# NOAA-GFDL/GRTCODE

Hardware: AMD Instinct MI355X
Metric: columns/sec (60-layer, 1 cm⁻¹ LBL, LW+SW) (higher is better)
Workload: dtype f64

## Files before the change

### grtcode_amd/csrc/grt_kernels.h

```cpp
#ifndef GRT_KERNELS_H_
#define GRT_KERNELS_H_

#include <stddef.h>
#include <stdint.h>

#ifdef __cplusplus
extern "C" {
#endif

#define GRT_MAX_ISO 18
#define GRT_MAX_SLOTS 53
#define GRT_MAX_TABLES 32

typedef struct GrtLineStore
{
    uint64_t n;
    double const *v0;
    double const *s0;
    float const *yair;
    float const *yself;
    float const *en;
    float const *nexp;
    float const *delta;
    uint8_t const *iso;
// ... 33 lines not shown
    GrtLineStore lines;
    GrtColumnLayout lay;
    double const *colstate;
    double const *tables;
    double const *h2o_tables;
    double w0, wres;
    uint64_t nw;
    int ncol;
    double *tau;
    uint64_t tau_col_stride;
    int tile;
    int nslice;
    int fast;
    float *gmom;
    uint64_t gmom_stride;
    int halo;
    int rcap;
    int tree_levels;
    int mom_terms;
    int profile_tag;
    int near_block;
    int deterministic;
    unsigned long long *probe;
    int direct_near;
    int tile_phase, tile_nphase;
    uint32_t const *tile_ranges;
    int lean;
    uint32_t const *tile_items;
    uint32_t n_items;
    GrtTableSpans spans;
    int *radius_table;
    int skip_tables;
    int narrow;
} GrtGasOpticsArgs;

typedef struct GrtContinua
{
    double const *colstate;
    uint64_t stride, off_cont, off_h2o;
    double const *tables;
    double const *h2o_tables;
    int num_tables, has_h2o_ctm;
    GrtTableSpans spans;
} GrtContinua;
int grt_launch_add_continua(void *stream, GrtContinua const *c, int num_layers, int ncol, uint64_t nw,
                            double *tau_gas, uint64_t col_stride);


int grt_launch_gas_optics(void *stream, GrtGasOpticsArgs const *a);
enum { GRT_TAG_FAR_OFFSET = 5 };
int grt_profile_begin(void *stream, int tag);
void grt_profile_end(void *stream, int slot);
int grt_launch_gas_optics_mp(void *stream, GrtGasOpticsArgs const *a);
int grt_gas_optics_mp_shape(GrtGasOpticsArgs const *a);
int grt_gas_optics_lean_shape(GrtGasOpticsArgs const *a);
int grt_tree_gather_by_wave(long long fsteps);
uint64_t grt_gas_optics_moment_floats(uint64_t nw, int levels, int terms);
double grt_gas_optics_moment_separation(int terms);

typedef struct GrtSweepBins
{
    double w0, wres;
    uint64_t num_wpoints, n;
    int ppb, do_interp, do_last_interp;
    double const *w;
    double *tau;
    uint64_t const *l, *r;
} GrtSweepBins;
int grt_launch_sweep_sort(void *stream, uint64_t n, int num_layers, double const *v0, double shift_max,
                          double const *lay, double const *prep, double *sorted);
int grt_launch_sweep(void *stream, int method, uint64_t n, int num_layers, double const *lines,
                     double const *ns, GrtSweepBins const *bins, double *tau);
int grt_launch_sweep_interpolate(void *stream, int num_layers, GrtSweepBins const *bins, double *tau);

int grt_launch_line_prep(void *stream, GrtGasOpticsArgs const *a, int col,
                         double *vnn, double *snn, double *gamma, double *alpha,
                         int64_t *win_s, int64_t *win_e);

int grt_launch_voigt_debug(void *stream, int fast, double w_start, uint64_t n, double wres, double center,
                           double gamma, double alpha, double *K_dev);

int grt_launch_rayleigh(void *stream, int num_layers, double w0, double dw, uint64_t nw,
                        double const *n_layer_host, double *tau, double *omega, double *g);

typedef struct GrtOpticsPtrs { double const *tau[8]; double const *omega[8]; double const *g[8]; } GrtOpticsPtrs;
int grt_launch_add_optics(void *stream, uint64_t n, int num_optics, GrtOpticsPtrs const *in,
                          double *tau, double *omega, double *g);

// ... 293 lines not shown
```

### grtcode_amd/csrc/hip/gas_optics_mp_dev.h

```cpp
#ifndef GRT_GAS_OPTICS_MP_DEV_H_
#define GRT_GAS_OPTICS_MP_DEV_H_
#include <type_traits>
#include "gas_optics_dev.h"

namespace {

constexpr int kMom = 8;
constexpr int kFarGradedMin = 64;
constexpr int kMomWide = 12;

__host__ __device__ inline double moment_separation(int terms)
{
    return terms == kMomWide ? 3.95 : 7.8;
}
constexpr size_t kLdsPerWorkgroup = 64*1024;
constexpr int kRcap = 12;
constexpr int kPowTable = 128;
constexpr int kCellLoop = 3;

template <int CTRL>
__device__ __forceinline__ float dpp_f(float v)
{
    int const b = __float_as_int(v);
    return __int_as_float(__builtin_amdgcn_update_dpp(0, b, CTRL, 0xf, 0xf, true));
}

__device__ __forceinline__ double row_pass(double v)
{
    int lo = __double2loint(v), hi = __double2hiint(v);
    lo = __builtin_amdgcn_update_dpp(lo, lo, 0x121, 0xf, 0xf, false);
    hi = __builtin_amdgcn_update_dpp(hi, hi, 0x121, 0xf, 0xf, false);
    return __hiloint2double(hi, lo);
}

// ... 108 lines not shown
    for (int i = 0; i < 8; ++i)
    {
        w[i] = dpp_add_by_bit<8>(g0[i], g1[i]);
    }
    float x[4];
#pragma unroll
    for (int i = 0; i < 4; ++i)
    {
        x[i] = dpp_add_by_bit<4>(w[i], w[i + 4]);
    }
    float y[2];
#pragma unroll
    for (int i = 0; i < 2; ++i)
    {
        float const keep = b1 ? x[i + 2] : x[i];
        float const send = b1 ? x[i] : x[i + 2];
        y[i] = keep + dpp_f<0x1B>(send);
    }
    float const keep = b0 ? y[1] : y[0];
    float const send = b0 ? y[0] : y[1];
    return keep + dpp_f<0xB1>(send);
}

constexpr int kRawCap = 128;
constexpr int kLeanListCap = 12;
constexpr int kLeanMaxP = 4;
constexpr int kLeanSlots = 16;
struct LeanTables
{
    float ps[kLeanSlots], p_ps[kLeanSlots], dop[kLeanSlots];
    float qn_m[kLeanSlots*GRT_MAX_ISO], qn_e[kLeanSlots*GRT_MAX_ISO];
    float ptab[kPowTable];
};
struct LeanRaw
{
    unsigned long long xl_mask[kWaves][kLeanListCap][kLeanMaxP];
    unsigned j[kWaves][kRawCap];
    float amp[kWaves][kRawCap];
    float delta[kWaves][kRawCap];
    unsigned idx[kWaves][kRawCap];
    unsigned xl_base[kWaves][kLeanListCap];
};

constexpr int kClasses = 3;
constexpr int kClassesSplit = 4;
constexpr int kMpQueue = 64;
constexpr int kMpQueueTree = 64;

template <int CAP, int NCLS>
struct MpQueue
{
    static constexpr int capacity = CAP;
    static constexpr int classes = NCLS;
    float amp[NCLS][kWaves][CAP];
    float xi[NCLS][kWaves][CAP];
    float y[NCLS][kWaves][CAP];
    unsigned short idx[NCLS][kWaves][CAP];
};
using MpQueueFlat = MpQueue<kMpQueue, kClassesSplit>;
using MpQueueTree = MpQueue<kMpQueueTree, kClassesSplit>;

__device__ __attribute__((noinline)) double exp_fp64_call(double x)
{
    return exp_fp64(x);
}

// ... 152 lines not shown
```

### grtcode_amd/csrc/hip/k_gas_optics_far.hip

```cpp
#include "gas_optics_mp_dev.h"

namespace {

__global__ __launch_bounds__(kBlock) void near_radius_kernel(GrtGasOpticsArgs a, long long fsteps_ll, int cell_shift, int ntiles)
{
    extern __shared__ __attribute__((aligned(16))) unsigned char smem[];
    double *ms_l = reinterpret_cast<double *>(smem);
    double *q_l = ms_l + 4*a.lay.num_slots;
    int const tid = threadIdx.x;
    int const layer = blockIdx.x, col = blockIdx.y;
    double const *cs = a.colstate + (uint64_t)col*a.lay.stride;
    double const *lay = cs + a.lay.off_lay + (uint64_t)layer*4;
    stage_column_state(a, cs, layer, ms_l, q_l, tid);
    __syncthreads();
    long long const nw = (long long)a.nw;
    for (int t = tid; t < ntiles; t += kBlock)
    {
        long long const c1 = ((long long)(t + 1) << cell_shift);
        bool um, cr;
        int const R = near_radius(a, lay, ms_l, (long long)t << cell_shift, c1 < nw ? c1 : nw, (int)fsteps_ll, &um, &cr);
        long long const F1 = c1 < nw ? c1 : nw;
        unsigned const tf = lean_tile_flags(a, lay, ms_l, (int)((long long)t << cell_shift), (int)F1, cr);
        a.radius_table[((uint64_t)col*a.lay.num_layers + layer)*ntiles + t] = R | (um ? 0x10000 : 0) | (cr ? 0x20000 : 0) | (int)(tf << kTileFlagsShift);
    }
}

__global__ __launch_bounds__(kBlock) void gas_optics_far_kernel(GrtGasOpticsArgs a, long long fsteps_ll, int cell_shift, int ncell)
{
    extern __shared__ __attribute__((aligned(16))) unsigned char smem[];
    int const fsteps = (int)fsteps_ll;
    double *acc = reinterpret_cast<double *>(smem);
    double *ms_l = acc + a.tile;
    double *q_l = ms_l + 4*a.lay.num_slots;
    float *mom = reinterpret_cast<float *>(q_l + GRT_MAX_ISO*a.lay.num_slots);
    float *invr = mom + (size_t)kMom*ncell;
    int *rtab = reinterpret_cast<int *>(invr + fsteps + 1);
    int const tid = threadIdx.x;
    int const layer = blockIdx.y, col = blockIdx.z;
    long long const nw = (long long)a.nw;
    long long const F0l = (long long)blockIdx.x*a.tile;
    long long const F1l = (F0l + a.tile < nw) ? F0l + a.tile : nw;
    int const F0 = (int)F0l, F1 = (int)F1l;
    double const *cs = a.colstate + (uint64_t)col*a.lay.stride;
    double const *lay = cs + a.lay.off_lay + (uint64_t)layer*4;
    double *out = a.tau + (uint64_t)col*a.tau_col_stride + (uint64_t)layer*a.nw;
    bool const own_radii = a.radius_table == nullptr || fsteps > kFarGradedMin;
    if (own_radii)
// ... 703 lines not shown
    return sizeof(double)*tile + sizeof(double)*num_slots*(4 + GRT_MAX_ISO) + sizeof(float)*((size_t)kMom*ncell + fsteps + 1)
           + sizeof(int)*((size_t)(ncell >> cell_shift) + 3);
}

}

extern "C" size_t grt_far_lds_bytes(int tile, int ncell, int fsteps, int num_slots, int cell_shift)
{
    return far_lds_bytes(tile, ncell, fsteps, num_slots, cell_shift);
}

extern "C" size_t grt_tree_lds_bytes(int tile, int num_slots, int ntab)
{
    return tree_lds_bytes(tile, num_slots, ntab);
}

extern "C" int grt_tree_gather_tile(void)
{
    return tree_gather_tile();
}

extern "C" int grt_tree_gather_ntab(int tile, int halo)
{
    return tree_gather_ntab(tile, halo);
}

extern "C" int grt_tree_gather_by_wave(long long fsteps)
{
    return tree_gather_by_wave(fsteps) ? 1 : 0;
}

extern "C" int grt_launch_near_radius(void *stream, GrtGasOpticsArgs const *bp, long long fsteps, int shift)
{
    int const ntiles = (int)((bp->nw + ((uint64_t)1 << shift) - 1) >> shift);
    hipLaunchKernelGGL(near_radius_kernel, dim3(bp->lay.num_layers, bp->ncol), dim3(kBlock),
                       sizeof(double)*bp->lay.num_slots*(4 + GRT_MAX_ISO), (hipStream_t)stream, *bp, fsteps, shift, ntiles);
    return (int)hipGetLastError();
}

extern "C" int grt_launch_far_field(void *stream, GrtGasOpticsArgs const *bp, long long fsteps, int shift)
{
    hipStream_t const s = (hipStream_t)stream;
    GrtGasOpticsArgs b = *bp;
    if (b.tree_levels > 0)
    {
        int first_level = 1;
        while ((2 << (first_level - 1)) <= b.tile && first_level <= b.tree_levels) ++first_level;
        if (b.mom_terms == kMomWide)
        {
            launch_tree<kMomWide>(s, b, fsteps, shift, first_level);
        }
        else
        {
            launch_tree<kMom>(s, b, fsteps, shift, first_level);
        }
        return (int)hipGetLastError();
    }
    int const far_want = 512;
    int far_tile = b.tile;
    while (2*far_tile <= far_want && (uint64_t)far_tile < b.nw
           && far_lds_bytes(2*far_tile, 2*far_tile + 2*(int)fsteps, (int)fsteps, b.lay.num_slots, shift) <= kLdsPerWorkgroup)
    {
        far_tile *= 2;
    }
    b.tile = far_tile;
    unsigned const far_tiles = (unsigned)((b.nw + far_tile - 1)/far_tile);
    int const far_ncell = far_tile + 2*(int)fsteps;
    hipLaunchKernelGGL(gas_optics_far_kernel, dim3(far_tiles, b.lay.num_layers, b.ncol), dim3(kBlock),
                       far_lds_bytes(far_tile, far_ncell, (int)fsteps, b.lay.num_slots, shift), s, b, fsteps, shift, far_ncell);
    return (int)hipGetLastError();
// ... 2 lines not shown
```

### grtcode_amd/csrc/hip/k_gas_optics_mp.hip

```cpp
#include "gas_optics_mp_dev.h"

extern "C" size_t grt_far_lds_bytes(int tile, int ncell, int fsteps, int num_slots, int cell_shift);
extern "C" size_t grt_tree_lds_bytes(int tile, int num_slots, int ntab);
extern "C" int grt_tree_gather_tile(void);
extern "C" int grt_tree_gather_ntab(int tile, int halo);
extern "C" int grt_tree_gather_by_wave(long long fsteps);
extern "C" int grt_launch_far_field(void *stream, GrtGasOpticsArgs const *b, long long fsteps, int shift);
extern "C" int grt_launch_near_radius(void *stream, GrtGasOpticsArgs const *b, long long fsteps, int shift);

namespace {

template <int CLASS, int ONLY, bool PACKED4, typename Queue>
__device__ __forceinline__ void drain_class(double *acc, Queue const *q, int wave, int first, int count, int lane)
{
    for (int i = first + lane; i < first + count; i += 64)
    {
        float const xi = q->xi[CLASS][wave][i], y = q->y[CLASS][wave][i];
        unsigned const idx = q->idx[CLASS][wave][i];
        float const far = (idx & 0x8000u) ? (y*kRsqrpi)*__builtin_amdgcn_rcpf(fmaf(xi, xi, y*y)) : 0.f;
        double const k = voigt_near<true, ONLY, PACKED4>(xi, y) - (double)far;
        GRT_ACC_ADD(&acc[idx & 0x7fffu], (double)q->amp[CLASS][wave][i]*k);
    }
}

// ... 75 lines not shown
            if (tid == 0)
            {
                probe_rec[2] = nlines;
                probe_rec[3] = (unsigned long long)R | ((unsigned long long)corrected << 16) | ((unsigned long long)use_moments << 17);
                probe_rec[1] = __builtin_readcyclecounter();
            }
        }
    };
    int const cell0 = TWO_PASS ? F0 : F0 - fsteps;
    int const A0 = TWO_PASS ? F0 - halo : F0;

    double const *cs = a.colstate + (uint64_t)col*a.lay.stride;
    double const *lay = cs + a.lay.off_lay + (uint64_t)layer*4;

    for (int i = tid; i < nacc; i += kBlock)
    {
        acc[i] = 0.0;
    }
    for (int i = tid; i < kMom*ncell; i += kBlock)
    {
        mom[i] = 0.f;
    }
    if (TREE && K == kMomWide && ncell == 0)
    {
        for (int i = tid; i < 2*(a.tile >> 5); i += kBlock)
        {
            occ_any[i] = 0u;
        }
    }
    for (int i = tid; i <= fsteps && !TWO_PASS; i += kBlock)
    {
        invr[i] = i > 0 ? 1.0f/(float)i : 0.f;
    }
    stage_column_state(a, cs, layer, ms_l, q_l, tid);
    for (int i = tid; i < kPowTable; i += kBlock)
    {
        ptab[i] = exp_fp64((double)((float)i/100.f)*lay[3]);
    }
    if (TWO_PASS && a.tile_ranges != nullptr)
    {
        if (tid == 0 && a.tile_items != nullptr)
        {
            range[0] = (long long)a.tile_items[4*(uint64_t)wi.group + 1];
            range[1] = (long long)a.tile_items[4*(uint64_t)wi.group + 2];
        }
        else if (tid == 0)
        {
            uint64_t const jlo = a.tile_ranges[2*tile_idx], jhi = a.tile_ranges[2*tile_idx + 1];
            uint64_t const per = (jhi - jlo + a.nslice - 1)/a.nslice;
            uint64_t const b = jlo + per*slice;
            uint64_t e = b + per;
            if (e > jhi) e = jhi;
            range[0] = (long long)(b < jhi ? b : jhi);
            range[1] = (long long)e;
        }
    }
    else if (wave == 0)
    {
        candidate_range_wave(a, lay, F0l, F1l, TWO_PASS ? 0 : fsteps_ll, slice, range, lane);
    }
    __syncthreads();
    if constexpr (PROBE)
    {
        if (tid == 0) probe_rec[11] = __builtin_readcyclecounter();
    }
    uint64_t const jbeg = (uint64_t)range[0];
    uint64_t const jend = (uint64_t)range[1];

    float const wres_f = (float)a.wres;
    double const inv_wres = 1./a.wres;
// ... 510 lines not shown
    bool const tree = a->tree_levels > 0;
    if ((items && (a->fast != 3 || a->tile_ranges == nullptr || a->n_items == 0 || tree || a->deterministic || a->probe != NULL))
        || (a->lean && (a->probe != NULL || !grt_gas_optics_lean_shape(a))) || (a->narrow && (a->fast != 3 || tree))
        || (a->near_block != 0 && (a->near_block != 64 || !tree)))
    {
        return (int)hipErrorInvalidValue;
    }
    unsigned long long const ngroups = items ? a->n_items : tiles*a->nslice;
    unsigned long long const blocks = ngroups*a->lay.num_layers*a->ncol;
    if (blocks == 0 || blocks > 0x7fffffffull)
    {
        return (int)hipErrorInvalidValue;
    }
    hipStream_t const s = (hipStream_t)stream;
    if (a->fast == 3)
    {
        int const halo = a->halo;
        int const nacc = a->tile + 2*halo, shift = log2_exact(a->tile);
        if (a->ncol > 65535 || a->lay.num_layers > 65535 || (tree && a->nslice != 1))
        {
            return (int)hipErrorInvalidValue;
        }
        hipError_t e = hipMemsetAsync(a->tau, 0, sizeof(double)*a->tau_col_stride*(size_t)a->ncol, s);
        if (e == hipSuccess && a->nslice > 1)
        {
            e = hipMemsetAsync(a->gmom, 0, sizeof(float)*a->gmom_stride*a->lay.num_layers*a->ncol, s);
        }
        bool const wide = tree && a->mom_terms == kMomWide;
        if (e != hipSuccess)
        {
            return (int)e;
        }
        GrtGasOpticsArgs b = *a;
        if (!tree && b.radius_table != nullptr)
        {
            int const rc_radius = grt_launch_near_radius(stream, &b, fsteps, shift);
            if (rc_radius != 0)
            {
                return rc_radius;
            }
        }
        int slot = a->profile_tag ? grt_profile_begin(stream, a->profile_tag) : -1;
        int const ncell = (tree && a->tile > kDirectTile) ? 0 : a->tile;
        size_t lds = mp_lds_bytes(nacc, ncell, 0, a->lay.num_slots, tree, tree && ncell == 0 ? a->tile : 0);
        if (a->lean)
        {
            lds += lean_lds_bytes(a->lay.num_slots);
        }
        int const nphase = a->deterministic ? (2*halo)/a->tile + 2 : 1;
        if (a->deterministic && a->nslice != 1)
        {
            return (int)hipErrorInvalidValue;
        }
        void (*first_pass)(GrtGasOpticsArgs, long long, unsigned, unsigned, int, int, int);
        if (wide && a->probe != NULL) first_pass = gas_optics_mp_probe_wide_kernel;
        else if (wide) first_pass = gas_optics_mp_kernel<true, true, kMomWide>;
        else if (tree) first_pass = gas_optics_mp_kernel_w5<true, true, kMom>;
        else if (a->probe != NULL) first_pass = a->narrow ? gas_optics_mp_probe_kernel<true> : gas_optics_mp_probe_kernel<false>;
        else if (a->lean) first_pass = a->narrow ? gas_optics_lean_kernel<true> : gas_optics_lean_kernel<false>;
        else first_pass = a->narrow ? gas_optics_mp_kernel_w5<true, false, kMom, true> : gas_optics_mp_kernel_w5<true, false, kMom>;
        for (int phase = 0; phase < nphase; ++phase)
        {
            b.tile_phase = phase;
            b.tile_nphase = nphase;
            hipLaunchKernelGGL(first_pass, dim3((unsigned)blocks), dim3(kBlock), lds, s, b, fsteps, (unsigned)ngroups,
                               golden_stride(ngroups), ncell, nacc, halo);
        }
        if (a->profile_tag) grt_profile_end(stream, slot);
        b.nslice = 1;
        slot = a->profile_tag ? grt_profile_begin(stream, a->profile_tag + GRT_TAG_FAR_OFFSET) : -1;
        int const rc_far = grt_launch_far_field(stream, &b, fsteps, shift);
        if (a->profile_tag) grt_profile_end(stream, slot);
        return rc_far;
    }
    int const ncell = a->tile + 2*(int)fsteps;
// ... 6 lines not shown
```

### grtcode_amd/csrc/hip/mp_lean_block.inc

```

    static_assert(kLeanP == 2, "the lean loop keeps the two lines of a lane in the halves of packed registers");
    constexpr int kLinesPerLane = LEAN_LOOP ? kLeanP : 1;
    [[maybe_unused]] bool lean_ok = false;
    [[maybe_unused]] LeanTables *lt = nullptr;
    [[maybe_unused]] LeanRaw *raw = nullptr;
    [[maybe_unused]] int rawcount = 0;
    [[maybe_unused]] int xcount = 0;
    [[maybe_unused]] float kh = 0.f, kl = 0.f, c2t = 0.f, pw = 0.f, pavg_f = 0.f, a_norm = 0.f, wres_v = 0.f, inv_wres_v = 0.f;
    [[maybe_unused]] unsigned tflags = 0u;
    auto uniform_flag = [](bool b) { return __builtin_amdgcn_readfirstlane((int)b) != 0; };
    if constexpr (LEAN_LOOP)
    {
        size_t const lean_off = ((size_t)(reinterpret_cast<unsigned char *>(invr + 1) - smem) + 15) & ~(size_t)15;
        lt = reinterpret_cast<LeanTables *>(smem + lean_off);
        raw = reinterpret_cast<LeanRaw *>(lt + 1);
        lean_ok = uniform_flag(a.lean != 0 && use_moments && R == 3 && fsteps >= 8 && halo >= 8
                               && a.lines.lean_a != nullptr);
        if (lean_ok)
        {
            for (int i = tid; i < a.lay.num_slots; i += kBlock)
            {
                lt->ps[i] = (float)ms_l[4*i];
                lt->p_ps[i] = (float)ms_l[4*i + 1];
                lt->dop[i] = (float)(((double)0.83255461115f/(double)kSqrln2)*ms_l[4*i + 3]);
            }
            for (int i = tid; i < a.lay.num_slots*GRT_MAX_ISO; i += kBlock)
            {
                double const v = q_l[i]*ms_l[(i/GRT_MAX_ISO)*4 + 2];
                int e = 0;
                double const m = frexp(v, &e);
                bool const ok = v > 0. && v < 1e300;
                lt->qn_m[i] = ok ? (float)(2.*m) : 0.f;
                lt->qn_e[i] = ok ? (float)(e - 1 - GRT_LEAN_S0_SHIFT) : 0.f;
            }
            for (int i = tid; i < kPowTable; i += kBlock)
            {
                lt->ptab[i] = (float)ptab[i];
            }
            __syncthreads();
            double const kTd = ((double)(-1.4387686f)*1.4426950408889634)*lay[2];
            kh = (float)kTd;
            kl = (float)(kTd - (double)kh);
            c2t = (float)((double)(-1.4387686f)*lay[2]);
            pw = (float)(lay[0]*inv_wres);
            pavg_f = (float)lay[0];
            a_norm = (float)(1./(3.14159265358979323846*a.wres));
            wres_v = wres_f;
            inv_wres_v = inv_wres_f;
            asm volatile("" : "+v"(kh), "+v"(kl), "+v"(c2t), "+v"(pw), "+v"(pavg_f), "+v"(a_norm), "+v"(wres_v), "+v"(inv_wres_v));
            unsigned const tf = tile_flags_known ? tile_flags : lean_tile_flags(a, lay, ms_l, F0, F1, corrected);
            tflags = (unsigned)__builtin_amdgcn_readfirstlane((int)tf);
        }
    }

    uint64_t const jal = lean_ok ? (jbeg & ~(uint64_t)1) : jbeg;
    uint64_t const walk_first = a.deterministic ? (wave == 0 ? jal : jend) : jal + (uint64_t)wave*64*kLinesPerLane;
    unsigned const walk_stride = (a.deterministic ? 64u : (unsigned)kBlock)*kLinesPerLane;

    [[maybe_unused]] auto drain_raw = [&](int const first, int const count)
    {
        if constexpr (LEAN_LOOP)
        {
            bool const on = lane < count;
            int const i = first + (on ? lane : 0);
            unsigned const packed = raw->idx[wave][i];
            unsigned const j = raw->j[wave][i];
            int const idx = (int)(packed & 4095u);
            int const c = idx + A0 - ((int)((packed >> 12) & 15u) - 3);
            double2 const lx = reinterpret_cast<double2 const *>(a.lines.lean_x)[j];
            float const yair = __int_as_float(__double2loint(lx.y)), yself = __int_as_float(__double2hiint(lx.y));
            double const *ms = ms_l + ((packed >> 16) & 63u)*4;
            double const wnoadj = lx.x + (double)raw->delta[wave][i]*lay[0];
            int const s = c - fsteps < 0 ? 0 : c - fsteps;
            LineWidths const lw = reference_widths(ptab[(packed >> 22) & 127u], yair, yself, ms, wnoadj);
            float const repwid = lw.repwid, y = lw.y;
            double const dwno = (double)s*a.wres + a.w0;
            float const xr = voigt_x(dwno, idx + A0 - s, a.wres, wnoadj, repwid);
            int const cls = on ? voigt_class<true, kSplit>(xr, y) : -1;
            queue_push(cls, raw->amp[wave][i]*(kRsqrpi*repwid), xr, y, (unsigned short)idx);
        }
    };
// ... 439 lines not shown
```

### grtcode_amd/csrc/host/grt_gas_launch.c

```c
#include <math.h>
#include <stdlib.h>
#include <string.h>
#include "grt_internal.h"

#define TREE_MIN_FSTEPS 200
#define ITEM_LINES 10000u

typedef struct LaunchPlan
{
    GrtGasOpticsArgs a;
    int tables;
    int items;
    double pmax;
    size_t moment_bytes;
    size_t radius_bytes;
    uint64_t probe_words;
} LaunchPlan;

static void auto_tune(GasOptics_t const *go, int ncol, int moments, int *tile, int *nslice)
{
    GrtGasOpticsImpl const *im = impl_of(go);
    uint64_t const nw = go->grid.n;
    double const per_cell = nw > 0 ? (double)im->store.n/(double)nw : 0.;
    int t = im->tile;
    if (t == 0)
    {
        int want = moments == 2 ? 256 : (moments ? 512 : 1024);
        while (moments == 2 && want > (ncol == 1 ? 128 : 64) && per_cell*(double)(want/2) >= 6000.
               && ((nw + want - 1)/want)*(uint64_t)go->num_layers*(uint64_t)ncol < 16384)
        {
            want >>= 1;
        }
        t = nw >= (uint64_t)want ? want : (int)(((nw + 63)/64)*64);
        if (moments == 2)
        {
            while (t & (t - 1))
            {
                t += 64;
            }
        }
    }
    int ns = im->nslice;
    if (ns == 0)
    {
        uint64_t const blocks = ((nw + t - 1)/t)*(uint64_t)go->num_layers*(uint64_t)ncol;
        double const per_tile = per_cell*(double)t;
        ns = 1;
        while (blocks*ns < 16384 && ns < 16 && per_tile/(double)(2*ns) >= 8000.)
// ... 242 lines not shown
            }
            a->gmom_stride = grt_gas_optics_moment_floats(a->nw, a->tree_levels, a->mom_terms);
        }
        if (!grt_gas_optics_mp_shape(a))
        {
            a->fast = im->fast == 3 ? 1 : 2;
            a->tree_levels = 0;
            a->mom_terms = 0;
            a->rcap = 12;
            if (a->fast == 1)
            {
                auto_tune(go, ncol, 1, &a->tile, &a->nslice);
                if (!grt_gas_optics_mp_shape(a))
                {
                    a->fast = 2;
                }
            }
        }
    }
    if (a->fast != 1 && a->fast != 3)
    {
        auto_tune(go, ncol, 0, &a->tile, &a->nslice);
    }
    a->direct_near = a->fast == 1 || a->fast == 3;
    uint64_t const tiles = (a->nw + (uint64_t)a->tile - 1)/(uint64_t)a->tile;
    if (a->fast == 3)
    {
        char const *lean = getenv("GRT_LEAN");
        a->lean = !(lean != NULL && lean[0] == '0') && grt_gas_optics_lean_shape(a);
        a->narrow = a->tree_levels == 0 && a->w0 + (double)a->nw*a->wres <= 4000.;
        a->near_block = a->tree_levels > 0 && grt_tree_gather_by_wave(fsteps) ? 64 : 0;
        p->moment_bytes = sizeof(float)*(size_t)a->gmom_stride*(size_t)go->num_layers;
        p->radius_bytes = a->tree_levels == 0 ? sizeof(int)*(size_t)tiles*(size_t)go->num_layers : 0;
        if (a->tree_levels == 0 || a->mom_terms == 12)
        {
            p->probe_words = 24*tiles*(uint64_t)a->nslice*(uint64_t)go->num_layers;
        }
        p->tables = im->sorted_v0_h != NULL && im->store.n > 0 && im->store.n < 0xffffffffull;
        for (int c = 0; c < ncol && p->tables && im->colstate_h != NULL; ++c)
        {
            double const *lay = im->colstate_h + (size_t)c*im->layout.stride + im->layout.off_lay;
            for (int i = 0; i < go->num_layers; ++i)
            {
                p->pmax = fabs(lay[(size_t)i*4]) > p->pmax ? fabs(lay[(size_t)i*4]) : p->pmax;
            }
        }
        char const *env = getenv("GRT_TILE_ITEMS");
        p->items = p->tables && im->nslice == 0 && a->tree_levels == 0 && !grt_deterministic()
                   && !(env != NULL && env[0] == '0') && tiles*(uint64_t)go->num_layers*(uint64_t)ncol < 16384;
    }
    if (grt_deterministic())
    {
        a->deterministic = 1;
        a->nslice = 1;
    }
}

static int grow(GasOptics_t *go, void **buf, size_t *have, size_t need)
{
    if (need > *have)
    {
        GRT_TRY(grt_dev_free(go->device, *buf));
        *buf = NULL;
        *have = 0;
        GRT_TRY(grt_dev_alloc(go->device, buf, need));
        *have = need;
    }
    return GRTCODE_SUCCESS;
}

static int bind(GasOptics_t *go, LaunchPlan const *p, int c0, int ncol, double *tau, uint64_t tau_col_stride,
                GrtGasOpticsArgs *a)
{
    GrtGasOpticsImpl *im = impl_of(go);
    *a = p->a;
    a->ncol = ncol;
    a->colstate = im->colstate_d + (size_t)c0*im->layout.stride;
    a->tau = tau + (size_t)c0*tau_col_stride;
    a->tau_col_stride = tau_col_stride;
    if (p->moment_bytes > 0)
    {
        GRT_TRY(grow(go, (void **)&im->gmom, &im->gmom_bytes, p->moment_bytes*(size_t)ncol));
        a->gmom = im->gmom;
    }
    if (p->radius_bytes > 0)
    {
        GRT_TRY(grow(go, (void **)&im->radius_table, &im->radius_bytes, p->radius_bytes*(size_t)ncol));
        a->radius_table = im->radius_table;
    }
    if (im->probe != NULL && p->probe_words > 0 && p->probe_words*(uint64_t)ncol <= im->probe_words)
    {
        a->probe = im->probe;
        a->lean = 0;
    }
    if (p->tables)
    {
        GRT_TRY(tile_tables(go, a, p->pmax));
        a->tile_ranges = im->tile_ranges_d;
        if (p->items && a->probe == NULL && im->n_items > 0)
        {
            a->tile_items = im->tile_items_d;
            a->n_items = im->n_items;
            a->nslice = im->items_cut > 1 ? 2 : 1;
        }
    }
    return GRTCODE_SUCCESS;
}

static int launch_sweep_columns(GasOptics_t *go, int ncol, double *tau_dev, uint64_t tau_col_stride)
{
    GrtGasOpticsImpl *im = impl_of(go);
    void *s = grt_dev_stream(go->device);
    int const L = go->num_layers;
    uint64_t nmax = 0;
    for (int sl = 0; sl < go->num_molecules; ++sl)
    {
        if (im->mstore[sl].n > nmax) nmax = im->mstore[sl].n;
    }
    if (nmax > 0 && im->sweep_scratch == NULL)
    {
        GRT_TRY(grt_dev_alloc(go->device, (void **)&im->sweep_scratch, sizeof(double)*8*(size_t)L*nmax));
    }
    GRT_TRY(grt_gas_optics_upload_states(go, ncol));
    GrtSweepBins bins = {go->bins.w0, go->bins.wres, go->bins.num_wpoints, go->bins.n, go->bins.ppb,
                         go->bins.do_interp, go->bins.do_last_interp, go->bins.w, go->bins.tau, go->bins.l, go->bins.r};
    int const method = go->optical_depth_method == wavenumber_sweep ? 0 : 1;
// ... 125 lines not shown
```

### grtcode_amd/csrc/host/grt_gas_optics.c

```c
#include <math.h>
#include <stdio.h>
#include <stdlib.h>
#include <string.h>
#include "grt_internal.h"
#include "grt_molecule_table.h"

static double const MIN_CUTOFF = 1.;
static double const MAX_CUTOFF = 50.;
static double const DEFAULT_CUTOFF = 25.;

static char const *const cfc_names[NUM_CFCS] = {
    "CFC-11", "CFC-12", "CFC-113", "CFC-114", "CFC-115", "HCFC-22", "HCFC-141b", "HCFC-142b",
    "HFC-23", "HFC-125", "HFC-134a", "HFC-143a", "HFC-152a", "HFC-227ea", "HFC-245fa", "CCl4",
    "C2F6", "CF4", "CH2Cl2", "NF3", "SF6"};

int grt_load_table_on_grid(char const *path, int expect_cols, SpectralGrid_t const *grid, fp_t *out)
{
    int rows = 0, cols = 0;
    char **tok = NULL;
    GRT_TRY(parse_csv(path, &rows, &cols, 1, &tok));
    int rc = GRTCODE_SUCCESS;
    fp_t *vals = malloc(sizeof(fp_t)*(size_t)rows*(size_t)cols);
    for (int i = 0; i < rows*cols; ++i)
    {
// ... 162 lines not shown
        if (told != im->fast)
        {
            told = im->fast;
            GRT_INFO("Line kernel form %d (%s); GRT_GAS_OPTICS_FAST=0 or grt_gas_optics_tune selects the reference's operation order.",
                     im->fast, im->fast == 0 ? "reference operation order, tau within 1e-11"
                               : "fused arithmetic, tau within 2e-6 of each layer's maximum, sums in the scheduler's order");
        }
    }
    size_t const V = (size_t)num_levels;
    go->x = calloc(NUM_MOLS*V, sizeof(fp_t));
    go->x_cfc = calloc(NUM_CFCS*V, sizeof(fp_t));
    go->x_cia = calloc(NUM_CIAS*V, sizeof(fp_t));
    GRT_TRY(grt_dev_alloc(go->device, (void **)&im->lin_tables, sizeof(double)*GRT_MAX_TABLES*grid->n));
    im->store_dirty = 1;
    GRT_TRY(inittips_d());
    GRT_INFO("Gas optics on device %d: %d levels, %zu grid points.", go->device, num_levels, (size_t)grid->n);
    return GRTCODE_SUCCESS;
}

EXTERN int destroy_gas_optics(GasOptics_t * const gas_optics)
{
    GRT_REQUIRE_PTR(gas_optics);
    GrtGasOpticsImpl *im = impl_of(gas_optics);
    if (im != NULL)
    {
        for (int i = 0; i < NUM_MOLS; ++i)
        {
            grt_free_host_lines(&im->host[i]);
        }
        GRT_TRY(grt_free_line_store(gas_optics));
        GRT_TRY(grt_dev_free(gas_optics->device, im->bins_block));
        GRT_TRY(grt_dev_free(gas_optics->device, im->gmom));
        GRT_TRY(grt_dev_free(gas_optics->device, im->radius_table));
        GRT_TRY(grt_dev_free(gas_optics->device, im->h2o_tables));
        GRT_TRY(grt_dev_free(gas_optics->device, im->lin_tables));
        GRT_TRY(grt_dev_free(gas_optics->device, im->colstate_d));
        GRT_TRY(grt_host_free_pinned(im->colstate_h));
        GRT_TRY(grt_dev_event_destroy(gas_optics->device, &im->colstate_uploaded));
        free(im);
    }
    free(gas_optics->h2o_cc.coefs);
    free(gas_optics->x);
    free(gas_optics->x_cfc);
    free(gas_optics->x_cia);
    gas_optics->impl = NULL;
    gas_optics->x = gas_optics->x_cfc = gas_optics->x_cia = NULL;
    gas_optics->h2o_cc.coefs = NULL;
    return GRTCODE_SUCCESS;
}

static int register_molecule(GasOptics_t *go, int molecule_id, GrtHostLines *lines, double w0, double wn)
{
    GrtGasOpticsImpl *im = impl_of(go);
    int const index = go->num_molecules;
    Molecule_t *mol = &go->mols[index];
    memset(mol, 0, sizeof(*mol));
    mol->id = molecule_id;
    mol->device = go->device;
    snprintf(mol->name, MOL_NAME_LEN, "%s", grt_molecule_table[molecule_id - 1].name);
    mol->mass = grt_molecule_table[molecule_id - 1].molar_mass;
    mol->mass /= 6.023e23;
    mol->num_isotopologues = grt_molecule_table[molecule_id - 1].num_iso;
    mol->line_params.num_lines = lines->n;
    mol->line_params.device = go->device;
    im->host[index] = *lines;
    memset(lines, 0, sizeof(*lines));
// ... 717 lines not shown
```

### grtcode_amd/csrc/host/grt_internal.h

```cpp
#ifndef GRT_INTERNAL_H_
#define GRT_INTERNAL_H_

#include <stddef.h>
#include <stdint.h>
#include "grtcode_hip_api.h"
#include "grt_ext.h"
#include "../grt_kernels.h"

void grt_err_begin(int code, char const *file, int line, char const *fmt, ...);
void grt_err_frame(char const *file, int line);
void grt_log(int level, char const *file, int line, char const *fmt, ...);

#define GRT_FAIL(code, ...) \
    do { grt_err_begin((code), __FILE__, __LINE__, __VA_ARGS__); return (code); } while (0)

#define GRT_TRY(expr) \
    do { int rc_ = (expr); if (rc_ != GRTCODE_SUCCESS) { grt_err_frame(__FILE__, __LINE__); return rc_; } } while (0)

#define GRT_REQUIRE_PTR(p) \
    do { if ((p) == NULL) GRT_FAIL(GRTCODE_NULL_ERR, "null pointer for argument '%s'.", #p); } while (0)

#define GRT_REQUIRE_RANGE(v, lo, hi) \
    do { double v_ = (double)(v), lo_ = (double)(lo), hi_ = (double)(hi); \
         if (v_ != v_) GRT_FAIL(GRTCODE_INVALID_ERR, "input value (%e) is Nan.", v_); \
// ... 45 lines not shown

typedef struct GrtHostLines
{
    uint64_t n;
    double *v0, *s0;
    float *yair, *yself, *en, *nexp, *delta;
    uint8_t *iso;
} GrtHostLines;

typedef struct GrtGasOpticsImpl
{
    GrtHostLines host[NUM_MOLS];
    int store_dirty;
    unsigned long store_tips_generation;
    GrtLineStore store;
    void *store_block;
    double *sorted_v0_h;
    uint32_t *tile_ranges_d;
    int tr_tile;
    uint64_t tr_tiles;
    double tr_pbound;
    uint32_t *tile_items_d;
    uint32_t *tile_items_h, *tile_ranges_h;
    uint32_t n_items;
    int items_cut;
    GrtLineStore mstore[NUM_MOLS];
    void *mstore_block[NUM_MOLS];
    double *sweep_scratch;
    void *bins_block;
    float *gmom;
    size_t gmom_bytes;
    int *radius_table;
    size_t radius_bytes;
    size_t scratch_cap_bytes;
    long long last_launch[8];
    double *h2o_tables;
    double *lin_tables;
    int num_lin;
    int lin_kind[GRT_MAX_TABLES];
    int lin_ref[GRT_MAX_TABLES];
    GrtTableSpans spans;
    int defer_tables;
    GrtColumnLayout layout;
    int layout_cols;
    double *colstate_h;
    void *colstate_uploaded;
    double *colstate_d;
    int tile, nslice, fast;
    int profile_tag;
    unsigned long long *probe;
    uint64_t probe_words;
} GrtGasOpticsImpl;
static inline GrtGasOpticsImpl *impl_of(GasOptics_t const *go) { return (GrtGasOpticsImpl *)go->impl; }

#define GRT_PRIVATE __attribute__((visibility("hidden")))

static inline size_t grt_align256(size_t x) { return (x + 255) & ~(size_t)255; }

int grt_gas_optics_prepare(GasOptics_t *go, int ncol);
int grt_gas_optics_wait_staging(GasOptics_t *go);
GRT_PRIVATE int grt_gas_optics_stage_column(GasOptics_t *go, fp_t const *p_mb, fp_t const *t);
GRT_PRIVATE int grt_gas_optics_upload_states(GasOptics_t *go, int ncol);
int grt_column_state(GasOptics_t const *go, fp_t const *p_mb, fp_t const *t,
                     fp_t const *x_mol , fp_t const *x_cfc ,
                     fp_t const *x_cia , double *dst);
int grt_gas_optics_defer_tables(GasOptics_t *go, int on);
// ... 30 lines not shown
```

Measured before the change: 624.4.

## Precompute per-layer lean tables in the radius kernel and copy them into the main kernel

The near-radius pre-pass, which runs once per (layer, column), now also builds the per-layer state, power table, lean float tables and scalars, and writes them as a LayerRecord in global memory. The lean gas-optics kernel then copies this record into LDS with 16-byte vector loads. Before, every workgroup recomputed the column-state staging, the exp-based power table and the frexp-based tables itself. This adds a global buffer and extra writes in the radius kernel, and enforces num_slots <= 16 whenever the record is used.

```diff
diff --git a/grtcode_amd/csrc/grt_kernels.h b/grtcode_amd/csrc/grt_kernels.h
--- a/grtcode_amd/csrc/grt_kernels.h
+++ b/grtcode_amd/csrc/grt_kernels.h
@@ -89,6 +89,7 @@
     int *radius_table;
     int skip_tables;
     int narrow;
+    void *layer_table;
 } GrtGasOpticsArgs;
 
 typedef struct GrtContinua
@@ -111,6 +112,7 @@
 int grt_launch_gas_optics_mp(void *stream, GrtGasOpticsArgs const *a);
 int grt_gas_optics_mp_shape(GrtGasOpticsArgs const *a);
 int grt_gas_optics_lean_shape(GrtGasOpticsArgs const *a);
+size_t grt_gas_optics_layer_record_bytes(void);
 int grt_tree_gather_by_wave(long long fsteps);
 uint64_t grt_gas_optics_moment_floats(uint64_t nw, int levels, int terms);
 double grt_gas_optics_moment_separation(int terms);
diff --git a/grtcode_amd/csrc/hip/gas_optics_mp_dev.h b/grtcode_amd/csrc/hip/gas_optics_mp_dev.h
--- a/grtcode_amd/csrc/hip/gas_optics_mp_dev.h
+++ b/grtcode_amd/csrc/hip/gas_optics_mp_dev.h
@@ -1,5 +1,6 @@
 #ifndef GRT_GAS_OPTICS_MP_DEV_H_
 #define GRT_GAS_OPTICS_MP_DEV_H_
+#include <cstddef>
 #include <type_traits>
 #include "gas_optics_dev.h"
 
@@ -174,6 +175,59 @@
     float qn_m[kLeanSlots*GRT_MAX_ISO], qn_e[kLeanSlots*GRT_MAX_ISO];
     float ptab[kPowTable];
 };
+__device__ __forceinline__ void lean_tables_fill(LeanTables *lt, double const *ms_l, double const *q_l, double const *ptab,
+                                                 int num_slots, int tid)
+{
+    for (int i = tid; i < num_slots; i += kBlock)
+    {
+        lt->ps[i] = (float)ms_l[4*i];
+        lt->p_ps[i] = (float)ms_l[4*i + 1];
+        lt->dop[i] = (float)(((double)0.83255461115f/(double)kSqrln2)*ms_l[4*i + 3]);
+    }
+    for (int i = tid; i < num_slots*GRT_MAX_ISO; i += kBlock)
+    {
+        double const v = q_l[i]*ms_l[(i/GRT_MAX_ISO)*4 + 2];
+        int e = 0;
+        double const m = frexp(v, &e);
+        bool const ok = v > 0. && v < 1e300;
+        lt->qn_m[i] = ok ? (float)(2.*m) : 0.f;
+        lt->qn_e[i] = ok ? (float)(e - 1 - GRT_LEAN_S0_SHIFT) : 0.f;
+    }
+    for (int i = tid; i < kPowTable; i += kBlock)
+    {
+        lt->ptab[i] = (float)ptab[i];
+    }
+}
+
+struct LeanScalars
+{
+    float kh, kl, c2t, pw, pavg_f, a_norm, wres, inv_wres;
+};
+__device__ __forceinline__ LeanScalars lean_scalars(double const *lay, double wres)
+{
+    double const inv_wres = 1./wres;
+    double const kTd = ((double)(-1.4387686f)*1.4426950408889634)*lay[2];
+    LeanScalars s;
+    s.kh = (float)kTd;
+    s.kl = (float)(kTd - (double)s.kh);
+    s.c2t = (float)((double)(-1.4387686f)*lay[2]);
+    s.pw = (float)(lay[0]*inv_wres);
+    s.pavg_f = (float)lay[0];
+    s.a_norm = (float)(1./(3.14159265358979323846*wres));
+    s.wres = (float)wres;
+    s.inv_wres = (float)inv_wres;
+    return s;
+}
+
+struct LayerRecord
+{
+    LeanTables lean;
+    LeanScalars scal;
+    double state[kLeanSlots*(4 + GRT_MAX_ISO) + kPowTable];
+};
+static_assert(sizeof(LeanTables) % 16 == 0 && sizeof(LeanScalars) == 32 && offsetof(LayerRecord, state) % 16 == 0
+              && sizeof(LayerRecord) % 16 == 0, "a workgroup copies the record's parts sixteen bytes per lane");
+
 struct LeanRaw
 {
     unsigned long long xl_mask[kWaves][kLeanListCap][kLeanMaxP];
diff --git a/grtcode_amd/csrc/hip/k_gas_optics_far.hip b/grtcode_amd/csrc/hip/k_gas_optics_far.hip
--- a/grtcode_amd/csrc/hip/k_gas_optics_far.hip
+++ b/grtcode_amd/csrc/hip/k_gas_optics_far.hip
@@ -7,12 +7,33 @@
     extern __shared__ __attribute__((aligned(16))) unsigned char smem[];
     double *ms_l = reinterpret_cast<double *>(smem);
     double *q_l = ms_l + 4*a.lay.num_slots;
+    double *ptab = q_l + GRT_MAX_ISO*a.lay.num_slots;
     int const tid = threadIdx.x;
     int const layer = blockIdx.x, col = blockIdx.y;
     double const *cs = a.colstate + (uint64_t)col*a.lay.stride;
     double const *lay = cs + a.lay.off_lay + (uint64_t)layer*4;
     stage_column_state(a, cs, layer, ms_l, q_l, tid);
+    if (a.layer_table != nullptr)
+    {
+        for (int i = tid; i < kPowTable; i += kBlock)
+        {
+            ptab[i] = exp_fp64((double)((float)i/100.f)*lay[3]);
+        }
+    }
     __syncthreads();
+    if (a.layer_table != nullptr)
+    {
+        LayerRecord *rec = static_cast<LayerRecord *>(a.layer_table) + ((uint64_t)col*a.lay.num_layers + layer);
+        for (int i = tid; i < a.lay.num_slots*(4 + GRT_MAX_ISO) + kPowTable; i += kBlock)
+        {
+            rec->state[i] = ms_l[i];
+        }
+        lean_tables_fill(&rec->lean, ms_l, q_l, ptab, a.lay.num_slots, tid);
+        if (tid == 0)
+        {
+            rec->scal = lean_scalars(lay, a.wres);
+        }
+    }
     long long const nw = (long long)a.nw;
     for (int t = tid; t < ntiles; t += kBlock)
     {
@@ -782,10 +803,19 @@
 
 extern "C" int grt_launch_near_radius(void *stream, GrtGasOpticsArgs const *bp, long long fsteps, int shift)
 {
+    if (bp->layer_table != nullptr && bp->lay.num_slots > kLeanSlots)
+    {
+        return (int)hipErrorInvalidValue;
+    }
     int const ntiles = (int)((bp->nw + ((uint64_t)1 << shift) - 1) >> shift);
     hipLaunchKernelGGL(near_radius_kernel, dim3(bp->lay.num_layers, bp->ncol), dim3(kBlock),
-                       sizeof(double)*bp->lay.num_slots*(4 + GRT_MAX_ISO), (hipStream_t)stream, *bp, fsteps, shift, ntiles);
+                       sizeof(double)*(bp->lay.num_slots*(4 + GRT_MAX_ISO) + kPowTable), (hipStream_t)stream, *bp, fsteps, shift, ntiles);
     return (int)hipGetLastError();
+}
+
+extern "C" size_t grt_gas_optics_layer_record_bytes(void)
+{
+    return sizeof(LayerRecord);
 }
 
 extern "C" int grt_launch_far_field(void *stream, GrtGasOpticsArgs const *bp, long long fsteps, int shift)
diff --git a/grtcode_amd/csrc/hip/k_gas_optics_mp.hip b/grtcode_amd/csrc/hip/k_gas_optics_mp.hip
--- a/grtcode_amd/csrc/hip/k_gas_optics_mp.hip
+++ b/grtcode_amd/csrc/hip/k_gas_optics_mp.hip
@@ -131,10 +131,37 @@
     {
         invr[i] = i > 0 ? 1.0f/(float)i : 0.f;
     }
-    stage_column_state(a, cs, layer, ms_l, q_l, tid);
-    for (int i = tid; i < kPowTable; i += kBlock)
-    {
-        ptab[i] = exp_fp64((double)((float)i/100.f)*lay[3]);
+    [[maybe_unused]] LayerRecord const *layer_rec = nullptr;
+    if constexpr (LEAN_LOOP)
+    {
+        if (a.layer_table != nullptr)
+        {
+            layer_rec = static_cast<LayerRecord const *>(a.layer_table) + ((uint64_t)col*a.lay.num_layers + layer);
+        }
+    }
+    if (LEAN_LOOP && layer_rec != nullptr)
+    {
+        static_assert(sizeof(Queue) % 16 == 0, "ms_l starts on a 16-byte boundary (nacc is even)");
+        int const nstate2 = (a.lay.num_slots*(4 + GRT_MAX_ISO) + kPowTable)/2;
+        double2 const *src = reinterpret_cast<double2 const *>(layer_rec->state);
+        for (int i = tid; i < nstate2; i += kBlock)
+        {
+            reinterpret_cast<double2 *>(ms_l)[i] = src[i];
+        }
+        size_t const lean_off = ((size_t)(reinterpret_cast<unsigned char *>(invr + 1) - smem) + 15) & ~(size_t)15;
+        float4 const *lsrc = reinterpret_cast<float4 const *>(&layer_rec->lean);
+        for (int i = tid; i < (int)(sizeof(LeanTables)/16); i += kBlock)
+        {
+            reinterpret_cast<float4 *>(smem + lean_off)[i] = lsrc[i];
+        }
+    }
+    else
+    {
+        stage_column_state(a, cs, layer, ms_l, q_l, tid);
+        for (int i = tid; i < kPowTable; i += kBlock)
+        {
+            ptab[i] = exp_fp64((double)((float)i/100.f)*lay[3]);
+        }
     }
     if (TWO_PASS && a.tile_ranges != nullptr)
     {
@@ -711,15 +738,20 @@
             return (int)e;
         }
         GrtGasOpticsArgs b = *a;
+        if (a->layer_table != nullptr && (!a->lean || tree || a->radius_table == nullptr))
+        {
+            return (int)hipErrorInvalidValue;
+        }
+        int slot = a->profile_tag ? grt_profile_begin(stream, a->profile_tag) : -1;
         if (!tree && b.radius_table != nullptr)
         {
             int const rc_radius = grt_launch_near_radius(stream, &b, fsteps, shift);
             if (rc_radius != 0)
             {
+                if (a->profile_tag) grt_profile_end(stream, slot);
                 return rc_radius;
             }
         }
-        int slot = a->profile_tag ? grt_profile_begin(stream, a->profile_tag) : -1;
         int const ncell = (tree && a->tile > kDirectTile) ? 0 : a->tile;
         size_t lds = mp_lds_bytes(nacc, ncell, 0, a->lay.num_slots, tree, tree && ncell == 0 ? a->tile : 0);
         if (a->lean)
diff --git a/grtcode_amd/csrc/hip/mp_lean_block.inc b/grtcode_amd/csrc/hip/mp_lean_block.inc
--- a/grtcode_amd/csrc/hip/mp_lean_block.inc
+++ b/grtcode_amd/csrc/hip/mp_lean_block.inc
@@ -18,35 +18,25 @@
                                && a.lines.lean_a != nullptr);
         if (lean_ok)
         {
-            for (int i = tid; i < a.lay.num_slots; i += kBlock)
-            {
-                lt->ps[i] = (float)ms_l[4*i];
-                lt->p_ps[i] = (float)ms_l[4*i + 1];
-                lt->dop[i] = (float)(((double)0.83255461115f/(double)kSqrln2)*ms_l[4*i + 3]);
-            }
-            for (int i = tid; i < a.lay.num_slots*GRT_MAX_ISO; i += kBlock)
-            {
-                double const v = q_l[i]*ms_l[(i/GRT_MAX_ISO)*4 + 2];
-                int e = 0;
-                double const m = frexp(v, &e);
-                bool const ok = v > 0. && v < 1e300;
-                lt->qn_m[i] = ok ? (float)(2.*m) : 0.f;
-                lt->qn_e[i] = ok ? (float)(e - 1 - GRT_LEAN_S0_SHIFT) : 0.f;
-            }
-            for (int i = tid; i < kPowTable; i += kBlock)
-            {
-                lt->ptab[i] = (float)ptab[i];
-            }
-            __syncthreads();
-            double const kTd = ((double)(-1.4387686f)*1.4426950408889634)*lay[2];
-            kh = (float)kTd;
-            kl = (float)(kTd - (double)kh);
-            c2t = (float)((double)(-1.4387686f)*lay[2]);
-            pw = (float)(lay[0]*inv_wres);
-            pavg_f = (float)lay[0];
-            a_norm = (float)(1./(3.14159265358979323846*a.wres));
-            wres_v = wres_f;
-            inv_wres_v = inv_wres_f;
+            LeanScalars ls;
+            if (layer_rec != nullptr)
+            {
+                ls = layer_rec->scal;
+            }
+            else
+            {
+                lean_tables_fill(lt, ms_l, q_l, ptab, a.lay.num_slots, tid);
+                __syncthreads();
+                ls = lean_scalars(lay, a.wres);
+            }
+            kh = ls.kh;
+            kl = ls.kl;
+            c2t = ls.c2t;
+            pw = ls.pw;
+            pavg_f = ls.pavg_f;
+            a_norm = ls.a_norm;
+            wres_v = ls.wres;
+            inv_wres_v = ls.inv_wres;
             asm volatile("" : "+v"(kh), "+v"(kl), "+v"(c2t), "+v"(pw), "+v"(pavg_f), "+v"(a_norm), "+v"(wres_v), "+v"(inv_wres_v));
             unsigned const tf = tile_flags_known ? tile_flags : lean_tile_flags(a, lay, ms_l, F0, F1, corrected);
             tflags = (unsigned)__builtin_amdgcn_readfirstlane((int)tf);
diff --git a/grtcode_amd/csrc/host/grt_gas_launch.c b/grtcode_amd/csrc/host/grt_gas_launch.c
--- a/grtcode_amd/csrc/host/grt_gas_launch.c
+++ b/grtcode_amd/csrc/host/grt_gas_launch.c
@@ -14,6 +14,7 @@
     double pmax;
     size_t moment_bytes;
     size_t radius_bytes;
+    size_t layer_bytes;
     uint64_t probe_words;
 } LaunchPlan;
 
@@ -322,6 +323,9 @@
         a->near_block = a->tree_levels > 0 && grt_tree_gather_by_wave(fsteps) ? 64 : 0;
         p->moment_bytes = sizeof(float)*(size_t)a->gmom_stride*(size_t)go->num_layers;
         p->radius_bytes = a->tree_levels == 0 ? sizeof(int)*(size_t)tiles*(size_t)go->num_layers : 0;
+        char const *layer_table = getenv("GRT_LAYER_TABLE");
+        p->layer_bytes = a->lean && p->radius_bytes > 0 && !(layer_table != NULL && layer_table[0] == '0')
+                         ? grt_gas_optics_layer_record_bytes()*(size_t)go->num_layers : 0;
         if (a->tree_levels == 0 || a->mom_terms == 12)
         {
             p->probe_words = 24*tiles*(uint64_t)a->nslice*(uint64_t)go->num_layers;
@@ -382,6 +386,11 @@
     {
         a->probe = im->probe;
         a->lean = 0;
+    }
+    if (p->layer_bytes > 0 && a->lean)
+    {
+        GRT_TRY(grow(go, &im->layer_table, &im->layer_bytes, p->layer_bytes*(size_t)ncol));
+        a->layer_table = im->layer_table;
     }
     if (p->tables)
     {
diff --git a/grtcode_amd/csrc/host/grt_gas_optics.c b/grtcode_amd/csrc/host/grt_gas_optics.c
--- a/grtcode_amd/csrc/host/grt_gas_optics.c
+++ b/grtcode_amd/csrc/host/grt_gas_optics.c
@@ -218,6 +218,7 @@
         GRT_TRY(grt_dev_free(gas_optics->device, im->bins_block));
         GRT_TRY(grt_dev_free(gas_optics->device, im->gmom));
         GRT_TRY(grt_dev_free(gas_optics->device, im->radius_table));
+        GRT_TRY(grt_dev_free(gas_optics->device, im->layer_table));
         GRT_TRY(grt_dev_free(gas_optics->device, im->h2o_tables));
         GRT_TRY(grt_dev_free(gas_optics->device, im->lin_tables));
         GRT_TRY(grt_dev_free(gas_optics->device, im->colstate_d));
diff --git a/grtcode_amd/csrc/host/grt_internal.h b/grtcode_amd/csrc/host/grt_internal.h
--- a/grtcode_amd/csrc/host/grt_internal.h
+++ b/grtcode_amd/csrc/host/grt_internal.h
@@ -101,6 +101,8 @@
     size_t gmom_bytes;
     int *radius_table;
     size_t radius_bytes;
+    void *layer_table;
+    size_t layer_bytes;
     size_t scratch_cap_bytes;
     long long last_launch[8];
     double *h2o_tables;
```

After: 627.6, median of 6. No clear change (+0.5%).
